# TobyBoyne/bark

Measured on AMD Instinct MI355X. Metric: forest-Gram + Cholesky MLL evals/sec at N=4096, 50 trees, higher is better.
Workload: dtype f64; 1 GPU; c3: N=4096 d=8 m=50, 256 prior forest samples per GPU (BASELINE configs[2]; sharding of configs[3]), noise U[0.05,0.15), mcmc_record_mll convention; N=4096, d=8, trees=50, forests_per_gpu=256, forests_total=256, chunk=256, parallelism=samples/1, launched_by=bench.py, device_wait=on

## Files before the change

bark_amd/csrc/chol_rows.h:

```cpp
#pragma once
#include "chol_diag.h"

namespace bark {
namespace {

template <int GEN>
__device__ __forceinline__ void form_tile(const f64x4 (&acc)[4][4], const Mats &p, int b, int rb, int cb, double *tile,
                                          double *lds, int tid, const Lane &q) {
    if (GEN == 0) {
#pragma unroll
        for (int mt = 0; mt < 4; ++mt)
#pragma unroll
            for (int v = 0; v < 4; ++v) {
                double *row = tile + (size_t)acc_row(q, mt, v) * p.ld;
#pragma unroll
                for (int nt = 0; nt < 4; ++nt) {
                    const int cc = acc_col(q, nt);
                    row[cc] = row[cc] - acc[mt][nt][v];
                }
            }
        return;
    }
    const int npad = p.nrb * NB;
    uint32_t *rows_l = reinterpret_cast<uint32_t *>(lds);
    uint32_t *cols_l = rows_l + p.nW * NB;
    const uint32_t *lb = p.leafx + (size_t)b * p.nW * npad;
    for (int e = tid; e < p.nW * NB; e += THREADS) {
        const int w = e >> 7, r = e & (NB - 1);
        rows_l[e] = lb[(size_t)w * npad + rb * NB + r];
        cols_l[e] = lb[(size_t)w * npad + cb * NB + r];
    }
    __syncthreads();
    const double inv_m = 1.0 / (double)p.m;
    const bool has_scale = p.scale != nullptr, has_shift = p.shift != nullptr;
    const double sc = has_scale ? p.scale[b] : 1.0;
    const double sh = has_shift ? p.shift[b] : 0.0;
    const double jitter = 1e-6 + p.noise[b];
#pragma unroll
    for (int mt = 0; mt < 4; ++mt) {
        uint32_t cnt[4][4] = {};
        for (int w = 0; w < p.nW; ++w) {
            uint32_t cw[4], rw[4];
#pragma unroll
            for (int nt = 0; nt < 4; ++nt) cw[nt] = cols_l[w * NB + acc_col(q, nt)];
#pragma unroll
            for (int v = 0; v < 4; ++v) rw[v] = rows_l[w * NB + acc_row(q, mt, v)];
#pragma unroll
            for (int v = 0; v < 4; ++v)
#pragma unroll
                for (int nt = 0; nt < 4; ++nt) cnt[v][nt] += code_count<(GEN > 0 ? GEN - 1 : 0)>(rw[v], cw[nt]);
        }
#pragma unroll
        for (int v = 0; v < 4; ++v) {
            const int r = acc_row(q, mt, v), gi = rb * NB + r;
            double *row = tile + (size_t)r * p.ld;
#pragma unroll
            for (int nt = 0; nt < 4; ++nt) {
                const int cc = acc_col(q, nt), gj = cb * NB + cc;
                double val;
                if (gi < p.N && gj < p.N) {
                    val = inv_m * (double)agree_count<(GEN > 0 ? GEN - 1 : 0)>(cnt[v][nt], p.m);
                    if (has_shift) val = val - sh;
                    if (has_scale) val = sc * val;
                    if (gi == gj) val = val + jitter;
                } else {
                    val = gi == gj ? 1.0 : 0.0;
                }
                row[cc] = val - acc[mt][nt][v];
            }
        }
    }
}

template <int NT>
__device__ __forceinline__ void y_partial(const f64x4 (&o)[NT], int rt, const double *__restrict__ z, double *part, int col0,
                                          const Lane &q) {
    double zr[4];
#pragma unroll
    for (int v = 0; v < 4; ++v) zr[v] = z[rt * 16 + q.lk + 4 * v];
#pragma unroll
    for (int nt = 0; nt < NT; ++nt) {
        double s = 0.0;
#pragma unroll
        for (int v = 0; v < 4; ++v) s = fma(o[nt][v], zr[v], s);
        s += __shfl_xor(s, 16);
        s += __shfl_xor(s, 32);
        if (q.lk == 0) part[rt * NB + col0 + nt * 16 + q.lr] = s;
    }
}
__device__ __forceinline__ void y_commit(const double *part, double *yi, int tid) {
    double s = part[tid];
#pragma unroll
    for (int rt = 1; rt < NSB_ROWS; ++rt) s += part[rt * NB + tid];
    yi[tid] = yi[tid] - s;
}

template <int GEN, int W>
__device__ __forceinline__ void syrk_tile(const Mats &p, int b, int cbk, const double *__restrict__ panel, int K, double *tile,
                                          double *lds, int tid, int lane, int lr, int lk) {
    using T = UpperBlocks<W>;
    f64x4 acc[9];
#pragma unroll
    for (int i = 0; i < 9; ++i) acc[i] = (f64x4){0.0, 0.0, 0.0, 0.0};
    constexpr int SK = 2 * BK;
    const int nk = K / SK;
    auto stage = [&](int kt, double *st) {
#pragma unroll
        for (int pp = 0; pp < SK / 4; ++pp) dma_row(panel + (size_t)(kt * SK + W + 4 * pp) * p.ld + lane * 2, st + (W + 4 * pp) * LDS_LD);
    };
    if (nk > 0) {
        stage(0, lds);
        asm volatile("s_waitcnt vmcnt(0)" ::: "memory");
        __syncthreads();
        for (int kt = 0; kt < nk; ++kt) {
            if (kt + 1 < nk) stage(kt + 1, lds + ((kt + 1) & 1) * (SK * LDS_LD));
            const double *st = lds + (kt & 1) * (SK * LDS_LD);
#pragma unroll
            for (int kk = 0; kk < SK / 4; ++kk) {
                double fr[8];
#pragma unroll
                for (int blk = 0; blk < 8; ++blk)
                    if (blk >= W) fr[blk] = st[(kk * 4 + lk) * LDS_LD + blk * 16 + lr];
#pragma unroll
                for (int i = 0; i < 9; ++i) acc[i] = __builtin_amdgcn_mfma_f64_16x16x4f64(fr[T::rb[i]], fr[T::cb[i]], acc[i], 0, 0, 0);
            }
            asm volatile("s_waitcnt vmcnt(0)" ::: "memory");
            __syncthreads();
        }
    }
    if (GEN == 0) {
#pragma unroll
        for (int i = 0; i < 9; ++i)
#pragma unroll
            for (int v = 0; v < 4; ++v) {
                double *e = tile + (size_t)(T::rb[i] * 16 + lk + 4 * v) * p.ld + T::cb[i] * 16 + lr;
                *e = *e - acc[i][v];
            }
        return;
    }
    const int npad = p.nrb * NB;
    uint32_t *codes = reinterpret_cast<uint32_t *>(lds);
    const uint32_t *lb = p.leafx + (size_t)b * p.nW * npad;
    for (int e = tid; e < p.nW * NB; e += THREADS) codes[e] = lb[(size_t)(e >> 7) * npad + cbk * NB + (e & (NB - 1))];
    __syncthreads();
    const double inv_m = 1.0 / (double)p.m;
    const bool has_scale = p.scale != nullptr, has_shift = p.shift != nullptr;
    const double sc = has_scale ? p.scale[b] : 1.0, sh = has_shift ? p.shift[b] : 0.0, jitter = 1e-6 + p.noise[b];
#pragma unroll
    for (int i = 0; i < 9; ++i) {
        uint32_t cnt[4] = {0, 0, 0, 0};
        for (int w = 0; w < p.nW; ++w) {
            const uint32_t cw = codes[w * NB + T::cb[i] * 16 + lr];
#pragma unroll
            for (int v = 0; v < 4; ++v) cnt[v] += code_count<(GEN > 0 ? GEN - 1 : 0)>(codes[w * NB + T::rb[i] * 16 + lk + 4 * v], cw);
        }
#pragma unroll
        for (int v = 0; v < 4; ++v) {
            const int r = T::rb[i] * 16 + lk + 4 * v, cc = T::cb[i] * 16 + lr, gi = cbk * NB + r, gj = cbk * NB + cc;
            double val;
            if (gi < p.N && gj < p.N) {
                val = inv_m * (double)agree_count<(GEN > 0 ? GEN - 1 : 0)>(cnt[v], p.m);
                if (has_shift) val = val - sh;
                if (has_scale) val = sc * val;
                if (gi == gj) val = val + jitter;
            } else {
                val = gi == gj ? 1.0 : 0.0;
            }
            tile[(size_t)r * p.ld + cc] = val - acc[i][v];
        }
    }
}

template <int GEN>
__global__ __launch_bounds__(THREADS, 2) void row_kernel(Mats p, int j, int kdone, int n_right, int n_tiles, int syrk) {
    extern __shared__ __attribute__((aligned(16))) double lds[];
    const int tid = threadIdx.x;
    int b, t;
    int rb, cb;
    if (syrk == 4) {
        const int first_diag = (int)xcd_grid(n_tiles, p.Bc), per = NXCD * ((p.Bc + NXCD - 1) / NXCD);
        if ((int)blockIdx.x >= first_diag) {
            const int local = (int)blockIdx.x - first_diag, which = local / per;
            b = local - which * per;
            if (b >= p.Bc) return;
            rb = cb = j + 1 + which;
        } else {
            if (!xcd_map(blockIdx.x, n_tiles, p.Bc, b, t)) return;
            if (t == 0) {
                rb = j;
                cb = j + 1;
            } else {
                rb = j + ((t - 1) & 1);
                cb = j + 2 + ((t - 1) >> 1);
            }
        }
    } else {
        if (syrk == 2) {
            const int first_diag = (int)xcd_grid(n_right, p.Bc);
            if ((int)blockIdx.x >= first_diag) {
                b = (int)blockIdx.x - first_diag;
                t = n_right;
                if (b >= p.Bc) return;
            } else if (!xcd_map(blockIdx.x, n_right, p.Bc, b, t)) {
                return;
            }
        } else if (!xcd_map(blockIdx.x, n_tiles, p.Bc, b, t)) {
            return;
        }
        rb = t < n_right ? j : j + 1;
        cb = t < n_right ? j + 1 + t : j + 1;
    }
    const Lane q = lane_of(tid);
    double *Ab = p.A + (size_t)b * p.bstride;
    if (syrk && rb == cb) {
        const int wsel = __builtin_amdgcn_readfirstlane(tid >> 6), lane = tid & 63;
        double *tile = Ab + (size_t)rb * NB * p.ld + (size_t)cb * NB;
        if (wsel == 0)
            syrk_tile<GEN, 0>(p, b, cb, Ab + (size_t)cb * NB, kdone * NB, tile, lds, tid, lane, q.lr, q.lk);
        else if (wsel == 1)
            syrk_tile<GEN, 1>(p, b, cb, Ab + (size_t)cb * NB, kdone * NB, tile, lds, tid, lane, q.lr, q.lk);
        else if (wsel == 2)
            syrk_tile<GEN, 2>(p, b, cb, Ab + (size_t)cb * NB, kdone * NB, tile, lds, tid, lane, q.lr, q.lk);
        else
            syrk_tile<GEN, 3>(p, b, cb, Ab + (size_t)cb * NB, kdone * NB, tile, lds, tid, lane, q.lr, q.lk);
        return;
    }
    f64x4 acc[4][4];
    zero_acc(acc);
    gemm_kmajor_dma(acc, Ab + (size_t)rb * NB, p.ld, Ab + (size_t)cb * NB, p.ld, kdone * NB, lds, tid, q);
    form_tile<GEN>(acc, p, b, rb, cb, Ab + (size_t)rb * NB * p.ld + (size_t)cb * NB, lds, tid, q);
}

__global__ __launch_bounds__(THREADS, 2) void panel_split_kernel(Mats p, int j, int n_right, int t_off, int n_tiles, int kb_lo,
                                                                  int kb_hi, int S, int s_off, int S_tot, double *slabs) {
    extern __shared__ __attribute__((aligned(16))) double lds[];
    const int tid = threadIdx.x;
    int b, ts;
    if (!xcd_map(blockIdx.x, n_tiles * S, p.Bc, b, ts)) return;
    const Lane q = lane_of(tid);
    const int tl = ts / S, s = ts - tl * S, t = t_off + tl;
    const int rb = t < n_right ? j : j + 1, cb = t < n_right ? j + 1 + t : j + 1;
    const long nkt = (long)(kb_hi - kb_lo) * (NB / BK);
    const int k0 = kb_lo * (NB / BK) + (int)((nkt * s) / S), k1 = kb_lo * (NB / BK) + (int)((nkt * (s + 1)) / S);
    const double *Ab = p.A + (size_t)b * p.bstride + (size_t)k0 * BK * p.ld;
    f64x4 acc[4][4];
    zero_acc(acc);
    gemm_kmajor_dma(acc, Ab + (size_t)rb * NB, p.ld, Ab + (size_t)cb * NB, p.ld, (k1 - k0) * BK, lds, tid, q);
    double *slab = slabs + ((size_t)((size_t)b * n_tiles + tl) * S_tot + s_off + s) * NB * NB;
#pragma unroll
    for (int mt = 0; mt < 4; ++mt)
#pragma unroll
        for (int v = 0; v < 4; ++v) {
            double *row = slab + (size_t)acc_row(q, mt, v) * NB;
#pragma unroll
            for (int nt = 0; nt < 4; ++nt) row[acc_col(q, nt)] = acc[mt][nt][v];
        }
}

#ifndef BARK_RED_ROWS
#define BARK_RED_ROWS 8
#endif
constexpr int RED_ROWS = BARK_RED_ROWS;
static_assert(RED_ROWS % 8 == 0 && NB % RED_ROWS == 0, "whole groups of 8 rows");
template <int GEN>
__global__ __launch_bounds__(THREADS) void panel_reduce_kernel(Mats p, int j, int n_right, int t_off, int n_tiles, int S,
                                                               const double *slabs) {
    const int tl = blockIdx.x / (NB / RED_ROWS), part = blockIdx.x % (NB / RED_ROWS), b = blockIdx.y;
    const int t = t_off + tl;
    const int rb = t < n_right ? j : j + 1, cb = t < n_right ? j + 1 + t : j + 1;
    const double inv_m = 1.0 / (double)p.m;
    const bool has_scale = GEN != 0 && p.scale != nullptr, has_shift = GEN != 0 && p.shift != nullptr;
    const double sc = has_scale ? p.scale[b] : 1.0, sh = has_shift ? p.shift[b] : 0.0, jitter = GEN != 0 ? 1e-6 + p.noise[b] : 0.0;
#pragma unroll
    for (int q = 0; q < RED_ROWS / 8; ++q) {
        const int e = (part * RED_ROWS + q * 8) * NB + 4 * threadIdx.x;
        const double *slab = slabs + (size_t)((size_t)b * n_tiles + tl) * S * NB * NB + e;
        f64x2 s0 = {0.0, 0.0}, s1 = {0.0, 0.0};
#pragma unroll 4
        for (int s = 0; s < S; ++s) {
            const f64x2 *src = reinterpret_cast<const f64x2 *>(slab + (size_t)s * NB * NB);
            s0 += src[0];
            s1 += src[1];
        }
        const int r = e >> 7, c0 = e & (NB - 1);
        f64x2 *dst = reinterpret_cast<f64x2 *>(p.A + (size_t)b * p.bstride + ((size_t)rb * NB + r) * p.ld + (size_t)cb * NB + c0);
        if (GEN == 0) {
            dst[0] -= s0;
            dst[1] -= s1;
            continue;
        }
        const int npad = p.nrb * NB, gi = rb * NB + r, gj0 = cb * NB + c0;
        const uint32_t *lb = p.leafx + (size_t)b * p.nW * npad;
        uint32_t cnt[4] = {0, 0, 0, 0};
        for (int w = 0; w < p.nW; ++w) {
            const uint32_t rw = lb[(size_t)w * npad + gi];
            const uint4 cw = *reinterpret_cast<const uint4 *>(lb + (size_t)w * npad + gj0);
            cnt[0] += code_count<(GEN > 0 ? GEN - 1 : 0)>(rw, cw.x);
            cnt[1] += code_count<(GEN > 0 ? GEN - 1 : 0)>(rw, cw.y);
            cnt[2] += code_count<(GEN > 0 ? GEN - 1 : 0)>(rw, cw.z);
            cnt[3] += code_count<(GEN > 0 ? GEN - 1 : 0)>(rw, cw.w);
        }
        double val[4];
#pragma unroll
        for (int i = 0; i < 4; ++i) {
            const int gj = gj0 + i;
            double v;
            if (gi < p.N && gj < p.N) {
                v = inv_m * (double)agree_count<(GEN > 0 ? GEN - 1 : 0)>(cnt[i], p.m);
                if (has_shift) v = v - sh;
                if (has_scale) v = sc * v;
                if (gi == gj) v = v + jitter;
            } else {
                v = gi == gj ? 1.0 : 0.0;
            }
            val[i] = v;
        }
        dst[0] = (f64x2){val[0], val[1]} - s0;
        dst[1] = (f64x2){val[2], val[3]} - s1;
    }
}

}
}
```

bark_amd/csrc/chol_tiles.h:

```cpp
#pragma once
#include "common.h"

namespace bark {
namespace {

#ifdef BARK_DIAG_STAMPS
__device__ unsigned long long g_diag_stamps[64];
#define DIAG_STAMP(i) do { if (blockIdx.x == 0 && threadIdx.x == 0) g_diag_stamps[i] = __builtin_readcyclecounter(); } while (0)
#else
#define DIAG_STAMP(i) do {} while (0)
#endif

typedef double f64x4 __attribute__((ext_vector_type(4)));
typedef double f64x2 __attribute__((ext_vector_type(2)));

constexpr int NB = TILE;
constexpr int BK = 16;
constexpr int LDS_LD = NB + 16;
constexpr int STAGE = 2 * BK * LDS_LD;
constexpr int GEMM_LDS_DOUBLES = 2 * STAGE;
constexpr int THREADS = 256;

struct Lane {
    int wr, wc, lr, lk;
};

__device__ __forceinline__ Lane lane_of(int tid) {
    Lane q;
    const int wave = tid >> 6, l = tid & 63;
    q.wr = wave >> 1;
    q.wc = wave & 1;
    q.lr = l & 15;
    q.lk = l >> 4;
    return q;
}

__device__ __forceinline__ int acc_row(const Lane &q, int mt, int v) { return q.wr * 64 + mt * 16 + q.lk + 4 * v; }
__device__ __forceinline__ int acc_col(const Lane &q, int nt) { return q.wc * 64 + nt * 16 + q.lr; }

__device__ __forceinline__ void zero_acc(f64x4 (&acc)[4][4]) {
#pragma unroll
    for (int mt = 0; mt < 4; ++mt)
#pragma unroll
        for (int nt = 0; nt < 4; ++nt) acc[mt][nt] = (f64x4){0.0, 0.0, 0.0, 0.0};
}

__device__ __forceinline__ void mma_stage(f64x4 (&acc)[4][4], const double *st, const Lane &q) {
    const double *As = st;
    const double *Bs = st + BK * LDS_LD;
#pragma unroll
    for (int kk = 0; kk < BK / 4; ++kk) {
        const double *ar = As + (kk * 4 + q.lk) * LDS_LD + q.wr * 64 + q.lr;
        const double *br = Bs + (kk * 4 + q.lk) * LDS_LD + q.wc * 64 + q.lr;
        const double a0 = ar[0], a1 = ar[16], a2 = ar[32], a3 = ar[48];
        const double b0 = br[0], b1 = br[16], b2 = br[32], b3 = br[48];
#define BARK_MFMA(mt, nt, av, bv) acc[mt][nt] = __builtin_amdgcn_mfma_f64_16x16x4f64(av, bv, acc[mt][nt], 0, 0, 0)
        BARK_MFMA(0, 0, a0, b0); BARK_MFMA(0, 1, a0, b1); BARK_MFMA(0, 2, a0, b2); BARK_MFMA(0, 3, a0, b3);
        BARK_MFMA(1, 0, a1, b0); BARK_MFMA(1, 1, a1, b1); BARK_MFMA(1, 2, a1, b2); BARK_MFMA(1, 3, a1, b3);
        BARK_MFMA(2, 0, a2, b0); BARK_MFMA(2, 1, a2, b1); BARK_MFMA(2, 2, a2, b2); BARK_MFMA(2, 3, a2, b3);
        BARK_MFMA(3, 0, a3, b0); BARK_MFMA(3, 1, a3, b1); BARK_MFMA(3, 2, a3, b2); BARK_MFMA(3, 3, a3, b3);
#undef BARK_MFMA
    }
}

typedef __attribute__((address_space(3))) void lds_ptr_t;
typedef const __attribute__((address_space(1))) void glb_ptr_t;

__device__ __forceinline__ void dma_row(const double *g, double *l) {
    __builtin_amdgcn_global_load_lds((glb_ptr_t *)g, (lds_ptr_t *)l, 16, 0, 0);
}

__device__ __forceinline__ void stage_dma(const double *__restrict__ A, long lda, const double *__restrict__ B,
                                          long ldb, int kt, double *st, int wave, int lane) {
    const double *a = A + ((long)kt * BK + wave) * lda + lane * 2;
    const double *b = B + ((long)kt * BK + wave) * ldb + lane * 2;
    double *as = st + wave * LDS_LD;
    double *bs = as + BK * LDS_LD;
#pragma unroll
    for (int p = 0; p < 4; ++p) {
        dma_row(a + (long)(4 * p) * lda, as + 4 * p * LDS_LD);
        dma_row(b + (long)(4 * p) * ldb, bs + 4 * p * LDS_LD);
    }
}

__device__ __forceinline__ void gemm_kmajor_dma(f64x4 (&acc)[4][4], const double *__restrict__ A, long lda,
                                                const double *__restrict__ B, long ldb, int K, double *lds, int tid,
                                                const Lane &q) {
    const int nk = K / BK;
    if (nk == 0) return;
    const int wave = __builtin_amdgcn_readfirstlane(tid >> 6), lane = tid & 63;
    stage_dma(A, lda, B, ldb, 0, lds, wave, lane);
    asm volatile("s_waitcnt vmcnt(0)" ::: "memory");
    __syncthreads();
    for (int kt = 0; kt < nk; ++kt) {
        if (kt + 1 < nk) stage_dma(A, lda, B, ldb, kt + 1, lds + ((kt + 1) & 1) * STAGE, wave, lane);
        mma_stage(acc, lds + (kt & 1) * STAGE, q);
        asm volatile("s_waitcnt vmcnt(0)" ::: "memory");
        __syncthreads();
    }
}


template <int DEF>
__device__ __forceinline__ void gemm_upper_tri(f64x4 (&acc)[4][4], const int (&rt)[4], const double *__restrict__ P,
                                               const double *__restrict__ T, long ldt, double *lds, int tid,
                                               const Lane &q) {
    constexpr int nd = DEF * (NB / BK), nk = nd + NB / BK;
    const int wave = __builtin_amdgcn_readfirstlane(tid >> 6), lane = tid & 63;
    stage_dma(P, NB, T, ldt, 0, lds, wave, lane);
    asm volatile("s_waitcnt vmcnt(0)" ::: "memory");
    __syncthreads();
    for (int kt = 0; kt < nd; ++kt) {
        stage_dma(P, NB, T, ldt, kt + 1, lds + ((kt + 1) & 1) * STAGE, wave, lane);
        const double *As = lds + (kt & 1) * STAGE;
        const double *Bs = As + BK * LDS_LD;
#pragma unroll
        for (int kk = 0; kk < BK / 4; ++kk) {
            const double *br = Bs + (kk * 4 + q.lk) * LDS_LD + q.wc * 64 + q.lr;
            const double b0 = br[0], b1 = br[16], b2 = br[32], b3 = br[48];
#pragma unroll
            for (int mt = 0; mt < 4; ++mt) {
                const double a = As[(kk * 4 + q.lk) * LDS_LD + rt[mt] * 16 + q.lr];
                acc[mt][0] = __builtin_amdgcn_mfma_f64_16x16x4f64(a, b0, acc[mt][0], 0, 0, 0);
                acc[mt][1] = __builtin_amdgcn_mfma_f64_16x16x4f64(a, b1, acc[mt][1], 0, 0, 0);
                acc[mt][2] = __builtin_amdgcn_mfma_f64_16x16x4f64(a, b2, acc[mt][2], 0, 0, 0);
                acc[mt][3] = __builtin_amdgcn_mfma_f64_16x16x4f64(a, b3, acc[mt][3], 0, 0, 0);
            }
        }
        asm volatile("s_waitcnt vmcnt(0)" ::: "memory");
        __syncthreads();
    }
#pragma unroll
    for (int kw = 0; kw < NB / BK; ++kw) {
        const int kt = nd + kw;
        if (kt + 1 < nk) stage_dma(P, NB, T, ldt, kt + 1, lds + ((kw + 1) & 1) * STAGE, wave, lane);
        const double *As = lds + (kw & 1) * STAGE;
        const double *Bs = As + BK * LDS_LD;
#pragma unroll
        for (int kk = 0; kk < BK / 4; ++kk) {
            const double *br = Bs + (kk * 4 + q.lk) * LDS_LD + q.wc * 64 + q.lr;
            const double b0 = br[0], b1 = br[16], b2 = br[32], b3 = br[48];
#pragma unroll
            for (int mt = 0; mt < 4; ++mt) {
                if (kw <= rt[mt]) {
                    const double a = As[(kk * 4 + q.lk) * LDS_LD + rt[mt] * 16 + q.lr];
                    acc[mt][0] = __builtin_amdgcn_mfma_f64_16x16x4f64(a, b0, acc[mt][0], 0, 0, 0);
                    acc[mt][1] = __builtin_amdgcn_mfma_f64_16x16x4f64(a, b1, acc[mt][1], 0, 0, 0);
                    acc[mt][2] = __builtin_amdgcn_mfma_f64_16x16x4f64(a, b2, acc[mt][2], 0, 0, 0);
                    acc[mt][3] = __builtin_amdgcn_mfma_f64_16x16x4f64(a, b3, acc[mt][3], 0, 0, 0);
                }
            }
        }
        asm volatile("s_waitcnt vmcnt(0)" ::: "memory");
        __syncthreads();
    }
}

constexpr int NXCD = 8;
__host__ __device__ __forceinline__ int xcd_rep(int Bc) {
    const int rounds = (Bc + NXCD - 1) / NXCD;
    if (Bc % NXCD == 0 || (Bc > NXCD && rounds * NXCD * 10 < Bc * 11)) return 1;
    return (Bc % 4 == 0) ? 2 : (Bc % 2 == 0) ? 4 : 8;
}
__host__ __device__ __forceinline__ bool xcd_map(int id, int ntiles, int Bc, int &b, int &tile) {
    const int R = xcd_rep(Bc), ntv = (ntiles + R - 1) / R;
    const int x = id % NXCD, q = id / NXCD;
    const int v = (q / ntv) * NXCD + x;
    b = v / R;
    tile = (q % ntv) * R + (v - b * R);
    return b < Bc && tile < ntiles;
}
__host__ __device__ inline unsigned xcd_grid(int ntiles, int Bc) {
    const int R = xcd_rep(Bc), ntv = (ntiles + R - 1) / R;
    return (unsigned)(NXCD * ((Bc * R + NXCD - 1) / NXCD) * ntv);
}

struct Mats {
    double *A;
    long ld, bstride;
    double *W;
    double *yz;
    double *accum;
    int32_t *info;
    int nrb;
    int ncb;
    int Bc;
    const uint32_t *leafx;
    const double *scale;
    const double *shift;
    const double *noise;
    int nW, m, N;
    int32_t *sync;
};

constexpr size_t W_STRIDE = (size_t)2 * NB * NB;
__device__ __forceinline__ double *w_block(const Mats &p, int b) { return p.W + (size_t)b * W_STRIDE + (size_t)NB * NB; }

}
}
```

Before: 2785 evals/s.

## Use wave-private LDS rings for row-update GEMM to drop per-stage barriers

Adds a GEMM path in which each wave DMA-loads its own 64-row slices of A and B into a private LDS ring and synchronises only through vmcnt waits, with no block-wide barrier per k-step. By default the row-update kernel now uses this path, while the split-panel kernel keeps the shared pipeline. The goal is to remove __syncthreads stalls on every stage. The cost is that each wave reloads the A/B data it would otherwise share with sibling waves, which doubles global/L2 traffic per tile. It also uses small 4-row k-stages with a software-pipelined operand read. Optional cycle-stamp instrumentation is included behind macros.

```diff
diff --git a/bark_amd/csrc/chol_rows.h b/bark_amd/csrc/chol_rows.h
--- a/bark_amd/csrc/chol_rows.h
+++ b/bark_amd/csrc/chol_rows.h
@@ -227,7 +227,11 @@
     }
     f64x4 acc[4][4];
     zero_acc(acc);
+#ifdef BARK_ROW_SHARED
     gemm_kmajor_dma(acc, Ab + (size_t)rb * NB, p.ld, Ab + (size_t)cb * NB, p.ld, kdone * NB, lds, tid, q);
+#else
+    gemm_kmajor_private(acc, Ab + (size_t)rb * NB, Ab + (size_t)cb * NB, p.ld, kdone * NB, lds, tid, q);
+#endif
     form_tile<GEN>(acc, p, b, rb, cb, Ab + (size_t)rb * NB * p.ld + (size_t)cb * NB, lds, tid, q);
 }
 
@@ -245,7 +249,11 @@
     const double *Ab = p.A + (size_t)b * p.bstride + (size_t)k0 * BK * p.ld;
     f64x4 acc[4][4];
     zero_acc(acc);
+#ifdef BARK_SPLIT_PRIVATE
+    gemm_kmajor_private(acc, Ab + (size_t)rb * NB, Ab + (size_t)cb * NB, p.ld, (k1 - k0) * BK, lds, tid, q);
+#else
     gemm_kmajor_dma(acc, Ab + (size_t)rb * NB, p.ld, Ab + (size_t)cb * NB, p.ld, (k1 - k0) * BK, lds, tid, q);
+#endif
     double *slab = slabs + ((size_t)((size_t)b * n_tiles + tl) * S_tot + s_off + s) * NB * NB;
 #pragma unroll
     for (int mt = 0; mt < 4; ++mt)
diff --git a/bark_amd/csrc/chol_tiles.h b/bark_amd/csrc/chol_tiles.h
--- a/bark_amd/csrc/chol_tiles.h
+++ b/bark_amd/csrc/chol_tiles.h
@@ -9,6 +9,19 @@
 #define DIAG_STAMP(i) do { if (blockIdx.x == 0 && threadIdx.x == 0) g_diag_stamps[i] = __builtin_readcyclecounter(); } while (0)
 #else
 #define DIAG_STAMP(i) do {} while (0)
+#endif
+
+#if defined(BARK_ROW_STAMPS) && defined(BARK_DIAG_STAMPS)
+#define ROW_STAMP_DECL unsigned long long rs_vm = 0, rs_bar = 0, rs_t, rs_t0 = __builtin_readcyclecounter()
+#define ROW_STAMP_BEGIN rs_t = __builtin_readcyclecounter()
+#define ROW_STAMP_END(acc) acc += __builtin_readcyclecounter() - rs_t
+#define ROW_STAMP_COMMIT do { if ((threadIdx.x & 63) == 0) { atomicAdd(&g_diag_stamps[32], rs_vm); atomicAdd(&g_diag_stamps[33], rs_bar); \
+        atomicAdd(&g_diag_stamps[34], (unsigned long long)(__builtin_readcyclecounter() - rs_t0)); atomicAdd(&g_diag_stamps[35], 1ull); } } while (0)
+#else
+#define ROW_STAMP_DECL do {} while (0)
+#define ROW_STAMP_BEGIN do {} while (0)
+#define ROW_STAMP_END(acc) do {} while (0)
+#define ROW_STAMP_COMMIT do {} while (0)
 #endif
 
 typedef double f64x4 __attribute__((ext_vector_type(4)));
@@ -92,12 +105,112 @@
     stage_dma(A, lda, B, ldb, 0, lds, wave, lane);
     asm volatile("s_waitcnt vmcnt(0)" ::: "memory");
     __syncthreads();
+    ROW_STAMP_DECL;
     for (int kt = 0; kt < nk; ++kt) {
         if (kt + 1 < nk) stage_dma(A, lda, B, ldb, kt + 1, lds + ((kt + 1) & 1) * STAGE, wave, lane);
         mma_stage(acc, lds + (kt & 1) * STAGE, q);
+        ROW_STAMP_BEGIN;
         asm volatile("s_waitcnt vmcnt(0)" ::: "memory");
+        ROW_STAMP_END(rs_vm);
+        ROW_STAMP_BEGIN;
         __syncthreads();
-    }
+        ROW_STAMP_END(rs_bar);
+    }
+    ROW_STAMP_COMMIT;
+}
+
+#ifndef BARK_PRIV_ROWS
+#define BARK_PRIV_ROWS 4
+#endif
+#ifndef BARK_PRIV_PIPE
+#define BARK_PRIV_PIPE 1
+#endif
+constexpr int PRIV_ROWS = BARK_PRIV_ROWS, PRIV_RING = 16 / PRIV_ROWS, PRIV_WAVE = 16 * LDS_LD;
+static_assert(PRIV_ROWS % 4 == 0 && PRIV_RING >= 2 && PRIV_RING * PRIV_ROWS == 16, "ring of whole MFMA k-steps, 16 rows per wave");
+static_assert(4 * PRIV_WAVE <= GEMM_LDS_DOUBLES, "wave-private rings fit the shared pipeline's LDS");
+
+#define BARK_WAIT_VMCNT(n) asm volatile("s_waitcnt vmcnt(%0)" ::"n"(n) : "memory")
+
+struct PrivOps {
+    double a[PRIV_ROWS / 4][4], b[PRIV_ROWS / 4][4];
+};
+__device__ __forceinline__ void read_private(PrivOps &o, const double *st, const Lane &q) {
+#pragma unroll
+    for (int kk = 0; kk < PRIV_ROWS / 4; ++kk) {
+        const double *ar = st + (kk * 4 + q.lk) * LDS_LD + q.lr;
+#pragma unroll
+        for (int i = 0; i < 4; ++i) {
+            o.a[kk][i] = ar[16 * i];
+            o.b[kk][i] = ar[64 + 16 * i];
+        }
+    }
+}
+__device__ __forceinline__ void mma_private(f64x4 (&acc)[4][4], const PrivOps &o) {
+#pragma unroll
+    for (int kk = 0; kk < PRIV_ROWS / 4; ++kk)
+#pragma unroll
+        for (int mt = 0; mt < 4; ++mt)
+#pragma unroll
+            for (int nt = 0; nt < 4; ++nt) acc[mt][nt] = __builtin_amdgcn_mfma_f64_16x16x4f64(o.a[kk][mt], o.b[kk][nt], acc[mt][nt], 0, 0, 0);
+}
+
+__device__ __forceinline__ void gemm_kmajor_private(f64x4 (&acc)[4][4], const double *__restrict__ A, const double *__restrict__ B,
+                                                    long ld, int K, double *lds, int tid, const Lane &q) {
+    const int nk = K / PRIV_ROWS;
+    if (nk == 0) return;
+    const int wave = __builtin_amdgcn_readfirstlane(tid >> 6), lane = tid & 63;
+    double *ring = lds + wave * PRIV_WAVE;
+    const double *g = (lane < 32 ? A + q.wr * 64 : B + q.wc * 64) + (lane & 31) * 2;
+    auto slot = [&](int kt) { return ring + (kt % PRIV_RING) * (PRIV_ROWS * LDS_LD); };
+    auto issue = [&](int kt) {
+        double *st = slot(kt);
+#pragma unroll
+        for (int r = 0; r < PRIV_ROWS; ++r) dma_row(g + r * ld, st + r * LDS_LD);
+        g += PRIV_ROWS * ld;
+    };
+    ROW_STAMP_DECL;
+#pragma unroll
+    for (int s = 0; s < PRIV_RING - 1; ++s)
+        if (s < nk) issue(s);
+#if BARK_PRIV_PIPE
+    PrivOps cur, nxt;
+    if (nk >= PRIV_RING - 1) BARK_WAIT_VMCNT((PRIV_RING - 2) * PRIV_ROWS);
+    else BARK_WAIT_VMCNT(0);
+    read_private(cur, slot(0), q);
+    for (int kt = 0; kt < nk; ++kt) {
+        ROW_STAMP_BEGIN;
+        if (kt + PRIV_RING - 1 < nk) {
+            asm volatile("s_waitcnt lgkmcnt(0)" ::: "memory");
+            issue(kt + PRIV_RING - 1);
+            BARK_WAIT_VMCNT((PRIV_RING - 2) * PRIV_ROWS);
+        } else {
+            BARK_WAIT_VMCNT(0);
+        }
+        ROW_STAMP_END(rs_vm);
+        if (kt + 1 < nk) read_private(nxt, slot(kt + 1), q);
+        mma_private(acc, cur);
+        cur = nxt;
+    }
+#else
+    for (int kt = 0; kt < nk; ++kt) {
+        ROW_STAMP_BEGIN;
+        if (kt + PRIV_RING - 1 < nk) {
+            asm volatile("s_waitcnt lgkmcnt(0)" ::: "memory");
+            issue(kt + PRIV_RING - 1);
+            BARK_WAIT_VMCNT((PRIV_RING - 1) * PRIV_ROWS);
+        } else {
+            BARK_WAIT_VMCNT(0);
+        }
+        ROW_STAMP_END(rs_vm);
+        PrivOps cur;
+        read_private(cur, slot(kt), q);
+        mma_private(acc, cur);
+    }
+#endif
+    ROW_STAMP_BEGIN;
+    __syncthreads();
+    ROW_STAMP_END(rs_bar);
+    ROW_STAMP_COMMIT;
 }
 
 
```

Measured after the change: 2634 evals/s. -5.4%, worse.

## Software-pipeline LDS fragment reads and interleave DMA issue with MFMA in k-major GEMM

Applied to the files above, without the earlier changes.

Rewrites the k-major GEMM inner loop to double-buffer register fragments loaded with inline-asm ds_read2_b64, waiting on lgkmcnt so LDS reads overlap the MFMA chain. The next-next stage's global-to-LDS DMA rows are issued one at a time between MFMAs of the last sub-step, with sched barriers pinning the order. It prefetches two stages ahead and keeps a single barrier per k-tile. This hides LDS latency and spreads DMA issue at the cost of hand-scheduled asm, fragile waitcnt accounting and more registers.

```diff
diff --git a/bark_amd/csrc/chol_tiles.h b/bark_amd/csrc/chol_tiles.h
--- a/bark_amd/csrc/chol_tiles.h
+++ b/bark_amd/csrc/chol_tiles.h
@@ -83,6 +83,74 @@
     }
 }
 
+#define BARK_SCHED_FENCE() __builtin_amdgcn_sched_barrier(0)
+
+struct Frag {
+    f64x2 a[2], b[2];
+};
+
+struct FragAddr {
+    unsigned a, b;
+};
+__device__ __forceinline__ FragAddr frag_addr(const double *lds, int a_col, int b_col, const Lane &q) {
+    const unsigned base = (unsigned)(size_t)(const __attribute__((address_space(3))) double *)lds;
+    FragAddr r;
+    r.a = base + (unsigned)((q.lk * LDS_LD + a_col + q.lr) * sizeof(double));
+    r.b = base + (unsigned)(((BK + q.lk) * LDS_LD + b_col + q.lr) * sizeof(double));
+    return r;
+}
+
+__device__ __forceinline__ void read_frag(Frag &f, const FragAddr &fa, unsigned stage_bytes, int kk) {
+    const unsigned off = stage_bytes + (unsigned)(kk * 4 * LDS_LD * sizeof(double));
+    asm volatile(
+        "ds_read2_b64 %0, %4 offset1:16\n\t"
+        "ds_read2_b64 %2, %5 offset1:16\n\t"
+        "ds_read2_b64 %1, %4 offset0:32 offset1:48\n\t"
+        "ds_read2_b64 %3, %5 offset0:32 offset1:48"
+        : "=&v"(f.a[0]), "=&v"(f.a[1]), "=&v"(f.b[0]), "=&v"(f.b[1])
+        : "v"(fa.a + off), "v"(fa.b + off)
+        : "memory");
+}
+template <int N>
+__device__ __forceinline__ void frag_wait(Frag &f) {
+    asm volatile("s_waitcnt lgkmcnt(%4)" : "+v"(f.a[0]), "+v"(f.a[1]), "+v"(f.b[0]), "+v"(f.b[1]) : "n"(N) : "memory");
+}
+__device__ __forceinline__ void tile_wait(Frag &f) {
+    asm volatile("s_waitcnt vmcnt(0) lgkmcnt(0)" : "+v"(f.a[0]), "+v"(f.a[1]), "+v"(f.b[0]), "+v"(f.b[1]) : : "memory");
+}
+
+struct StageRows {
+    const double *a, *b;
+    long lda, ldb;
+    double *as;
+    __device__ __forceinline__ StageRows(const double *__restrict__ A, long lda_, const double *__restrict__ B, long ldb_, int kt,
+                                         double *st, int wave, int lane)
+        : a(A + ((long)kt * BK + wave) * lda_ + lane * 2), b(B + ((long)kt * BK + wave) * ldb_ + lane * 2), lda(lda_), ldb(ldb_),
+          as(st + wave * LDS_LD) {}
+    __device__ __forceinline__ void issue(int r) const {
+        const int p = r >> 1;
+        if (r & 1)
+            dma_row(b + (long)(4 * p) * ldb, as + (BK + 4 * p) * LDS_LD);
+        else
+            dma_row(a + (long)(4 * p) * lda, as + 4 * p * LDS_LD);
+    }
+};
+
+template <bool DMA>
+__device__ __forceinline__ void mma_step(f64x4 (&acc)[4][4], const Frag &f, const StageRows *rows, bool more) {
+#pragma unroll
+    for (int mt = 0; mt < 4; ++mt)
+#pragma unroll
+        for (int h = 0; h < 2; ++h) {
+            acc[mt][2 * h] = __builtin_amdgcn_mfma_f64_16x16x4f64(f.a[mt >> 1][mt & 1], f.b[h][0], acc[mt][2 * h], 0, 0, 0);
+            acc[mt][2 * h + 1] = __builtin_amdgcn_mfma_f64_16x16x4f64(f.a[mt >> 1][mt & 1], f.b[h][1], acc[mt][2 * h + 1], 0, 0, 0);
+            if (DMA) {
+                if (more) rows->issue(2 * mt + h);
+                BARK_SCHED_FENCE();
+            }
+        }
+}
+
 __device__ __forceinline__ void gemm_kmajor_dma(f64x4 (&acc)[4][4], const double *__restrict__ A, long lda,
                                                 const double *__restrict__ B, long ldb, int K, double *lds, int tid,
                                                 const Lane &q) {
@@ -92,12 +160,36 @@
     stage_dma(A, lda, B, ldb, 0, lds, wave, lane);
     asm volatile("s_waitcnt vmcnt(0)" ::: "memory");
     __syncthreads();
+    const FragAddr fa = frag_addr(lds, q.wr * 64, q.wc * 64, q);
+    constexpr unsigned SB = STAGE * sizeof(double);
+    Frag f0, f1;
+    read_frag(f0, fa, 0, 0);
+    if (nk > 1) stage_dma(A, lda, B, ldb, 1, lds + STAGE, wave, lane);
     for (int kt = 0; kt < nk; ++kt) {
-        if (kt + 1 < nk) stage_dma(A, lda, B, ldb, kt + 1, lds + ((kt + 1) & 1) * STAGE, wave, lane);
-        mma_stage(acc, lds + (kt & 1) * STAGE, q);
-        asm volatile("s_waitcnt vmcnt(0)" ::: "memory");
+        const unsigned st = (kt & 1) * SB;
+        read_frag(f1, fa, st, 1);
+        frag_wait<4>(f0);
+        BARK_SCHED_FENCE();
+        mma_step<false>(acc, f0, nullptr, false);
+        BARK_SCHED_FENCE();
+        read_frag(f0, fa, st, 2);
+        frag_wait<4>(f1);
+        BARK_SCHED_FENCE();
+        mma_step<false>(acc, f1, nullptr, false);
+        BARK_SCHED_FENCE();
+        read_frag(f1, fa, st, 3);
+        frag_wait<4>(f0);
+        BARK_SCHED_FENCE();
+        mma_step<false>(acc, f0, nullptr, false);
+        BARK_SCHED_FENCE();
+        tile_wait(f1);
         __syncthreads();
-    }
+        read_frag(f0, fa, SB - st, 0);
+        BARK_SCHED_FENCE();
+        const StageRows rows(A, lda, B, ldb, kt + 2, lds + (kt & 1) * STAGE, wave, lane);
+        mma_step<true>(acc, f1, &rows, kt + 2 < nk);
+    }
+    asm volatile("s_waitcnt lgkmcnt(0)" : "+v"(f0.a[0]), "+v"(f0.a[1]), "+v"(f0.b[0]), "+v"(f0.b[1]) : : "memory");
 }
 
 
```

Result: no change. 2831 evals/s before, 2836 evals/s after, median of 6 (+0.1%).
